# corelab-src/dacapo

Hardware: AMD Instinct MI355X
Metric: NTT/s (NTT-equivalents over one run() of the ResNet HEVM program, nt=2^14) (higher is better)
Workload: dtype u64; 1 GPU; ResNet-20 (SiLU) HEVM program traced from the reference's examples/benchmarks/ResNet.py with its resnet20.silu.model weights, nt=2^14 slots, N=2^15, 14 x 60-bit primes (SEAL_HEVM.cpp:39-53); one independent ciphertext stream per GPU; streams_per_gpu=1, parallelism=replicas x1 (no collective in the op path)

## Files before the change

### dacapo_amd/csrc/hevm_vm.hip

```cpp
#include "hevm_vm.hpp"

#include "../../include/dacapo_ckks.h"
#include "c_api_types.hpp"
#include "chacha.hpp"
#include "seal_serial.hpp"

#include <math.h>
#include <string.h>
#include <sys/random.h>

#include <algorithm>
#include <cmath>
#include <chrono>
#include <fstream>
#include <iostream>

namespace dacapo {

constexpr int kVmThreads = 256;

constexpr int kRngCoefs = 8;

__device__ __forceinline__ int rng_cbd(u64 w)
{
// ... 393 lines not shown
        abort();
    }
    const int bits = (int)option(OPT_PRIME_BITS);
    ctx.reset(new Context(logN, K, bits, primes, ksp, alpha));
    ctx->ensure_scratch();
    encoder.reset(new HostEncoder(logN));
    use_plan = option(OPT_PLAN) != 0;
    plan_graph = option(OPT_PLAN_GRAPH) != 0;
    plan_dag = option(OPT_PLAN_GRAPH) == 2;
    plan_lanes = option(OPT_PLAN_LANES) >= 2 ? 2 : 1;
    host_encoder = option(OPT_HOST_ENCODER) != 0;
    fold_rescale_into_boot = option(OPT_FOLD_RESCALE_BOOT) != 0;
    lazy_sums = option(OPT_HYB_LAZY_SUM) != 0;
    double_hoist = (lazy_sums && option(OPT_HYB_DOUBLE_HOIST) != 0) || ks_lazy == 2;
    max_batch = std::max(1, (int)option(OPT_MAX_BATCH));
    chain_fusion = option(OPT_CHAIN_FUSION) != 0;
    secret_weight = (int)option(OPT_SECRET_HW);
    boot_secret_weight = (int)option(OPT_BOOT_SECRET_HW);
    rot_compose = option(OPT_ROT_COMPOSE) != 0;
    online_encode = option(OPT_ONLINE_ENCODE) != 0 && use_plan && !host_encoder;
    lanes.resize(1);
    DC_HIP_CHECK(hipStreamCreateWithFlags(&lanes[0].stream, hipStreamNonBlocking));
    lanes[0].ws = ctx->ws0;
    lanes[0].boot_plain.d = dalloc((size_t)ctx->max_level() * ctx->N);
    lanes[0].boot_plain.level = ctx->max_level();
    DC_HIP_CHECK(vm_malloc(&d_epoch, 8));
    DC_HIP_CHECK(hipMemset(d_epoch, 0, 8));
    cur = 0;
}

// ... 1228 lines not shown
    const CrtTables &tb = crt_tables(ell);
    u64 *pt = W().ks_tmp;
    u64 *lohi = W().ks_digits;
    f_irows_decrypt(c, src, keys.sk, ell, pt, S());
    launch_ntt_cols_inv(c, pt, (long)N, ell, nullptr, 0, 0, S());
    const CrtDev cd{ tb.inv, tb.mmod, tb.hmod, tb.hdig, tb.mdbl };
    DC_LAUNCH(reencode_kernel, dim3((unsigned)((N / 2 + kVmThreads) / kVmThreads)), dim3(kVmThreads), 0, S(), lohi,
                       lohi + N, pt, ell, N, c.d_mods, cd, new_scale / src_scale);
    Plain ptx{ lanes[cur].boot_plain.d, target_level, new_scale };
    DC_LAUNCH(lift_i128_kernel, dim3((unsigned)(N / kVmThreads), (unsigned)target_level), dim3(kVmThreads), 0, S(),
                       ptx.d, lohi, lohi + N, N, c.d_mods);
    launch_ntt(c, false, ptx.d, (long)N, target_level, nullptr, 0, 0, S());
    encrypt_plain(dst, ptx);
}

void HEVM::plan_zero_encrypt(int first, int B, int t, hipStream_t s)
{
    Context &c = *ctx;
    const size_t N = c.N;
    const int cnt = t + 1;
    if (!keys.pk) {
        fprintf(stderr, "[dacapo_amd] bootstrap: this VM has no public key\n");
        abort();
    }
    Plan &P = plan;
    DC_LAUNCH(sample_enc_batch_kernel, dim3((unsigned)(N / (kRngCoefs * kVmThreads)), (unsigned)(3 * B)), dim3(kVmThreads), 0, s,
                       P.boot_ue, N, cnt, rng.secret, ((u64)1 << 32) + (u64)first, c.d_mods, d_epoch);
    launch_ntt(c, false, P.boot_ue, (long)N, 3 * cnt * B, nullptr, 0, cnt, s);
    DC_LAUNCH(pk_encrypt_batch_kernel, dim3((unsigned)(N / (2 * kVmThreads)), (unsigned)cnt, (unsigned)(2 * B)), dim3(kVmThreads),
                       0, s, P.boot_tmp, keys.pk, (long)c.K * (long)N, P.boot_ue, cnt, N, c.d_mods);
    b_rescale(c, P.ws[0], P.d_boot_rs + first, B, cnt, s);
}

void HEVM::plan_boot_step(int first, int B, int ell, int t, int lane, hipStream_t s, const Handoff &h)
{
    Context &c = *ctx;
    const size_t N = c.N;
    if (!keys.sk) {
        fprintf(stderr, "[dacapo_amd] bootstrap: needs a full VM (secret + public key)\n");
        abort();
    }
    Plan &P = plan;
    const BootItem *items = P.d_boot + first;
    const CrtTables &tb = crt_tables(ell);
    const CrtDev cd{ tb.inv, tb.mmod, tb.hmod, tb.hdig, tb.mdbl };
    u64 *pt = P.boot_pt[lane], *ptx = P.boot_ptx[lane];
// ... 26 lines not shown
    case 9: op_mulcp(op.dst, op.lhs, op.rhs); break;
    case 10: op_bootstrap(op.dst, op.lhs, op.rhs); break;
    case kOpConj: op_conj(op.dst, op.lhs); break;
    case kOpModRaise: op_modraise(op.dst, op.lhs, op.rhs); break;
    case kOpSetScale: op_setscale(op.dst, op.lhs, op.rhs); break;
    case kOpKeySwitch: op_keyswitch(op.dst, op.lhs, op.rhs); break;
    default: break;
    }
}

void HEVM::execute()
{
    memset(op_counts, 0, sizeof(op_counts));
    n_keyswitch = n_ntt = 0;
    n_hops = n_decomp = 0, n_fold = 0;
    t_bootstrap = 0.0;
    int i = (int)((header.hevm_header_size + config.config_body_length) / 8), j = 0;
    for (const WireOp &op : ops) {
        if (debug) {
            std::cout << std::endl;
            std::cout << std::oct << i++ << " " << std::dec << j++ << std::endl;
            std::cout << "opcode [" << op.opcode << "], dst [" << op.dst << "], lhs [" << op.lhs << "], rhs [" << op.rhs << "]"
                      << std::endl;
        }
        if (op.opcode <= 10) op_counts[op.opcode]++;
        if (op.opcode == 0 || (op.opcode > 10 && (op.opcode < kOpConj || op.opcode > kOpKeySwitch))) continue;
        dispatch(op);
    }
    bump_epoch(S());
}
// ... 351 lines not shown
    if (ntts) *ntts = h->n_ntt;
}

void hevm_last_run_hoist_stats(void *vm, int64_t *hops, int64_t *decompositions)
{
    auto h = V(vm);
    if (hops) *hops = h->n_hops;
    if (decompositions) *decompositions = h->n_decomp;
}

void hevm_last_run_fold_rescale_stats(void *vm, int64_t *pairs)
{
    if (pairs) *pairs = V(vm)->n_fold;
}

int64_t hevm_plan_lazy_groups(void *vm, int32_t *out, int64_t cap)
{
    auto h = V(vm);
    if (!h->plan.ready) return -1;
    std::vector<int32_t> flat;
    for (const auto &p : h->plan.pops)
        if (!p.dead && p.kind == HEVM::P_ROTSUM) {
            flat.push_back((int32_t)p.ops.size());
            flat.insert(flat.end(), p.ops.begin(), p.ops.end());
        }
    if (out && cap >= (int64_t)flat.size()) memcpy(out, flat.data(), flat.size() * sizeof(int32_t));
    return (int64_t)flat.size();
}

void hevm_destroy(void *vm)
// ... 11 lines not shown
```

### dacapo_amd/csrc/hevm_vm.hpp

```cpp
#pragma once
#include "wire_parse.hpp"
#include <complex>
#include <deque>
#include <map>
#include <set>
#include <memory>
#include <string>
#include <unordered_set>
#include <vector>

#include "../../include/hevm_abi.h"
#include "chacha.hpp"
#include "seal_serial.hpp"
#include "kernels.hpp"
#include "encoder.hpp"
#include "plan.hpp"

namespace dacapo {

struct VmAllocs {
    std::unordered_set<void *> live;
};
extern thread_local VmAllocs *g_vm_allocs;
template <class T>
// ... 125 lines not shown
        bool dead = false;
        int wave = 0, step = -1;
        int op = -1;
        bool direct = false;
        std::vector<u32> elts;
        std::vector<const u64 *> keys;
        std::vector<int> ops;
        std::vector<int> plains;
    };
    struct Step {
        PopKind kind;
        int level = 0, first = 0, count = 0;
        int target = 0;
        int wave = 0, lane = 0;
        Handoff h;
        int fused_consumer = -1;
        bool fold_rs = false;
        int gfirst = 0, gcount = 0;
        int unique = 0;
        std::vector<const u64 *> reads, writes;
    };
    struct Plan {
        bool ready = false;
        std::vector<Val> vals;
        std::vector<Pop> pops;
        std::vector<Step> steps;
        std::vector<int> final_val;
        KsItem *d_ks = nullptr;
        MulItem *d_mul = nullptr;
        MulRsItem *d_mulrs = nullptr;
// ... 6 lines not shown
        CtView *d_cont_other = nullptr;
        struct EncGroup { int wave, level, first, count; u64 *out; };
        std::vector<EncGroup> enc_groups;
        EncItem *d_enc_items = nullptr;
        u64 *enc_arena = nullptr;
        double2 *enc_scratch = nullptr;
        int *d_enc_overflow = nullptr;
        size_t enc_arena_bytes = 0, enc_scratch_bytes = 0;
        std::vector<EwItem> h_ew;
        std::vector<u64 *> handoff_bufs;
        size_t n_fused = 0;
        BootItem *d_boot = nullptr;
        RsItem *d_boot_rs = nullptr;
        size_t zenc_bytes = 0;
        u64 *zenc = nullptr, *boot_ue = nullptr, *boot_tmp = nullptr, *boot_pt[2] = { nullptr, nullptr }, *boot_ptx[2] = { nullptr, nullptr };
        struct BootChunk { int first, count, target; };
        std::vector<BootChunk> boot_chunks;
        BatchWs ws[2];
        std::vector<hipEvent_t> events;
        std::vector<u64 *> pool;
        int64_t n_keyswitch = 0, n_ntt = 0;
        int64_t n_hops = 0, n_decomp = 0;
        int64_t n_fold = 0;
        size_t launches = 0, max_live = 0;
        hipGraph_t graph = nullptr;
        hipGraphExec_t graph_exec = nullptr;
    } plan;
    bool plan_graph = true;
    bool plan_dag = false;
    void capture_plan();
    bool capture_plan_dag();
    void issue_step(const Step &st, hipStream_t q);
    void drop_plan_graph();
    void issue_plan(hipStream_t s);
    bool use_plan = true;
    bool test_zero_enc = false;
    int max_batch = 64;
    std::vector<u64 *> home;
    int streams = 1, sel = 0;
    std::vector<u64 *> reg_base;
    void set_streams(int n);
    void select_stream(int s);
    void build_plan();
    void run_plan();
    void boot_item(CtView src, int src_level, double src_scale, hevm_ctxt &dst, int target_level);
    void plan_zero_encrypt(int first, int B, int t, hipStream_t s);
    void plan_boot_step(int first, int B, int ell, int t, int lane, hipStream_t s, const Handoff &h);
    bool rot_compose = false;
    std::vector<int> compose_rotation(int steps) const;
    mutable std::vector<int> rot_offsets;
    mutable std::set<int> rot_offset_set;
    mutable size_t rot_offsets_epoch = (size_t)-1;
    int boot_secret_weight = 0;
    int secret_weight = 0;
    bool ks_hoist = false;
    int ks_lazy = 0;
    bool ks_fold_rescale = false;
    KsItem *d_hoist_items = nullptr;
    void rotate_hop_vm(CtView dst, CtView src, u32 elt, const u64 *key, int ell);
    bool chain_fusion = true;
    hipStream_t aux_stream = nullptr;
    bool double_hoist = false;
    double *dh_consts = nullptr;
    std::map<int, EncItem> dh_items;
    void ensure_special_limbs(const std::vector<int> &plain_regs);
    bool lazy_sums = false;
    bool fold_rescale_into_boot = false;
    int plan_lanes = 2;
    void bump_epoch(hipStream_t s);

    int64_t op_counts[11] = { 0 };
    int64_t n_keyswitch = 0, n_ntt = 0;
    int64_t n_hops = 0, n_decomp = 0;
    int64_t n_fold = 0;
    double t_bootstrap = 0.0;

    VmAllocs allocs;
    HEVM() { g_vm_allocs = &allocs; }
    void destroy_device_state();
    size_t key_elems() const { return (size_t)ctx->key_digits() * 2 * ctx->K * ctx->N; }
    void init_context(int logN, int K, const u64 *primes, int dir_ksp = 0, int dir_alpha = 0);
    void generate_keys(const RngKeys &rng, bool secret, bool pub, bool eval);
    void gen_kswitch_key(u64 *key, const u64 *new_key, u64 key_id);
    void gen_kswitch_key_in(Context &c, u64 *key, const u64 *key_sk, const u64 *new_key, u64 key_id);
    void fill_sparse_secret(u64 *dst, int weight, u32 domain);
    void generate_boot_switch_keys();
    size_t swk_down_elems() const { return (size_t)2 * (1 + ctx->ksp) * ctx->N; }
    void add_galois_key(u32 elt);
    void save_keys(const std::string &dir);
// ... 37 lines not shown
```

### dacapo_amd/csrc/options.cpp

```cpp
#include "options.hpp"

#include "../../include/hevm_abi.h"

#include <stdio.h>
#include <stdlib.h>
#include <string.h>

namespace dacapo {

struct OptDef {
    const char *name;
    long long def;
};
static const OptDef kDefs[OPT_COUNT] = {
    { "logn", 15 },
    { "primes", 14 },
    { "prime_bits", 60 },
    { "ks_special", 1 },
    { "ks_alpha", 0 },
    { "secret_hw", 0 },
    { "boot_secret_hw", 0 },
    { "rot_compose", 0 },
    { "plan", 1 },
    { "plan_graph", 1 },
    { "plan_lanes", 2 },
    { "plan_aux_min_cost", 3 },
    { "max_batch", 64 },
    { "chain_fusion", 1 },
    { "host_encoder", 0 },
    { "online_encode", 0 },
    { "fold_rescale_boot", 0 },
    { "hyb_mfma", 1 },
    { "hyb_fuse", 2 },
    { "hyb_lazy_sum", 0 },
    { "hyb_double_hoist", 0 },
    { "ks_hoist", 0 },
    { "ks_lazy_sum", 0 },
    { "ks_fold_rescale", 0 },
    { "seal_compr", 0 },
    { "trace", 0 },
    { "step_profile", 0 },
    { "small_tile_wgs", -1 },
// ... 129 lines not shown
```

### dacapo_amd/csrc/options.hpp

```cpp
#pragma once

namespace dacapo {

enum Opt : int {
    OPT_LOGN,
    OPT_PRIMES,
    OPT_PRIME_BITS,
    OPT_KS_SPECIAL,
    OPT_KS_ALPHA,
    OPT_SECRET_HW,
    OPT_BOOT_SECRET_HW,
    OPT_ROT_COMPOSE,
    OPT_PLAN,
    OPT_PLAN_GRAPH,
    OPT_PLAN_LANES,
    OPT_PLAN_AUX_MIN_COST,
    OPT_MAX_BATCH,
    OPT_CHAIN_FUSION,
    OPT_HOST_ENCODER,
    OPT_ONLINE_ENCODE,
    OPT_FOLD_RESCALE_BOOT,
    OPT_HYB_MFMA,
    OPT_HYB_FUSE,
    OPT_HYB_LAZY_SUM,
    OPT_HYB_DOUBLE_HOIST,
    OPT_KS_HOIST,
    OPT_KS_LAZY_SUM,
    OPT_KS_FOLD_RESCALE,
    OPT_SEAL_COMPR,
    OPT_TRACE,
    OPT_STEP_PROFILE,
    OPT_SMALL_TILE_WGS,
// ... 25 lines not shown
```

### dacapo_amd/csrc/plan_exec.hip

```cpp
#include <math.h>
#include <string.h>

#include <algorithm>
#include <chrono>
#include <map>
#include <functional>
#include <queue>
#include <set>
#include <tuple>

#include "hevm_vm.hpp"

namespace dacapo {

#define ks_ntts(ell) ks_ntt_count(c, (ell))

template <class T>
static T *upload(const std::vector<T> &v)
{
    T *d = nullptr;
    DC_HIP_CHECK(vm_malloc(&d, std::max<size_t>(v.size(), 1) * sizeof(T)));
    if (!v.empty()) DC_HIP_CHECK(hipMemcpy(d, v.data(), v.size() * sizeof(T), hipMemcpyHostToDevice));
    return d;
}

void HEVM::build_plan()
{
    Context &c = *ctx;
    const size_t N = c.N;
    Plan &P = plan;
    for (u64 *b : P.handoff_bufs) (void)vm_free(b);
    P.handoff_bufs.clear();
    for (void *p : { (void *)P.d_enc_items, (void *)P.enc_arena, (void *)P.enc_scratch, (void *)P.d_enc_overflow })
        if (p) (void)vm_free(p);
    P.d_enc_items = nullptr, P.enc_arena = nullptr, P.enc_scratch = nullptr, P.d_enc_overflow = nullptr;
    P.enc_groups.clear(), P.enc_arena_bytes = P.enc_scratch_bytes = 0;
    if (P.d_cont_other) (void)vm_free(P.d_cont_other), P.d_cont_other = nullptr;
    if (P.d_mulrs) (void)vm_free(P.d_mulrs), P.d_mulrs = nullptr;
    for (void *p : { (void *)P.d_ks, (void *)P.d_mul, (void *)P.d_rs, (void *)P.d_ew, (void *)P.d_sum, (void *)P.d_sum_srcs, (void *)P.d_sumg, (void *)P.d_sumg_srcs, (void *)P.d_boot,
                     (void *)P.d_boot_rs, (void *)P.zenc, (void *)P.boot_ue, (void *)P.boot_tmp, (void *)P.boot_pt[0], (void *)P.boot_ptx[0],
                     (void *)P.boot_pt[1], (void *)P.boot_ptx[1] })
        if (p) (void)vm_free(p);
    P.d_boot = nullptr, P.d_boot_rs = nullptr, P.zenc = P.boot_ue = P.boot_tmp = nullptr;
    P.boot_pt[0] = P.boot_pt[1] = P.boot_ptx[0] = P.boot_ptx[1] = nullptr;
    P.boot_chunks.clear();
    if (P.graph_exec) (void)hipGraphExecDestroy(P.graph_exec);
    if (P.graph) (void)hipGraphDestroy(P.graph);
    P.graph_exec = nullptr, P.graph = nullptr;
    P.vals.clear(), P.pops.clear(), P.steps.clear();
    P.n_keyswitch = P.n_ntt = 0;
    P.n_hops = P.n_decomp = 0, P.n_fold = 0;
    const size_t nreg = ciphers.size();
    const int S = streams;
    std::vector<int> cur(nreg, -1);
    auto new_val = [&](int level, double scale) {
        Val v;
        v.level = level, v.scale = scale, v.root = (int)P.vals.size();
        P.vals.push_back(v);
        return (int)P.vals.size() - 1;
    };
// ... 529 lines not shown
            if (!ok) continue;
            bp = order;
            if (B.fold_rs) {
                std::vector<int> &rs = fold_pops.at(bi);
                for (size_t k = 0; k < bp.size(); k++) rs[k] = fold_rs_of.at(bp[k]);
            }
            Step &A = P.steps[(size_t)ai];
            A.fused_consumer = (int)bi;
            A.h.cont = B.kind == P_RESCALE ? CONT_RS : B.kind == P_BOOT ? CONT_BOOT : CONT_MUL;
            if (B.kind == P_MULCC)
                for (size_t k = 0; k < bp.size(); k++) mul_fused_src[(size_t)bp[k]] = which2[k];
            P.n_fused++;
        }
    }
    if (plan_lanes >= 2) {
        auto cost = [](const Step &st) { return st.kind == P_ROT || st.kind == P_MULCC || st.kind == P_ROTSUM ? 8 : st.kind == P_BOOT ? 5 : st.kind == P_RESCALE ? 3 : 1; };
        for (size_t a = 0; a < P.steps.size();) {
            size_t b = a;
            while (b < P.steps.size() && P.steps[b].wave == P.steps[a].wave) b++;
            std::vector<size_t> idx;
            for (size_t i = a; i < b; i++) idx.push_back(i);
            std::stable_sort(idx.begin(), idx.end(), [&](size_t x, size_t y) { return cost(P.steps[x]) > cost(P.steps[y]); });
            int load[2] = { 0, 0 };
            for (size_t i : idx) {
                const int lane = load[1] < load[0] ? 1 : 0;
                P.steps[i].lane = lane, load[lane] += cost(P.steps[i]);
            }
            if (load[1] < (int)option(OPT_PLAN_AUX_MIN_COST))
                for (size_t i = a; i < b; i++) P.steps[i].lane = 0;
            a = b;
        }
// ... 363 lines not shown
        for (int pi : step_pops[s]) {
            const Pop &p = O[(size_t)pi];
            for (int v : p.srcs) st.reads.push_back(V[(size_t)V[(size_t)v].root].buf);
            st.writes.push_back(V[(size_t)V[(size_t)p.dst].root].buf);
        }
        if (st.fold_rs)
            for (int pi : fold_pops.at(s)) st.writes.push_back(V[(size_t)V[(size_t)O[(size_t)pi].dst].root].buf);
        if (st.fused_consumer >= 0 && st.h.cont == CONT_MUL)
            for (int pi : step_pops[(size_t)st.fused_consumer])
                for (int v : O[(size_t)pi].srcs) st.reads.push_back(V[(size_t)V[(size_t)v].root].buf);
        for (auto *vec : { &st.reads, &st.writes }) {
            std::sort(vec->begin(), vec->end());
            vec->erase(std::unique(vec->begin(), vec->end()), vec->end());
        }
    }
    if (!h_boot_pops.empty()) {
        const size_t nb = h_boot_pops.size(), slot = (size_t)2 * boot_tmax * N;
        DC_HIP_CHECK(vm_malloc(&P.zenc, nb * slot * sizeof(u64)));
        P.zenc_bytes = nb * slot * sizeof(u64);
        std::vector<int> order(nb);
        for (size_t i = 0; i < nb; i++) order[i] = (int)i;
        std::stable_sort(order.begin(), order.end(), [&](int a, int b) {
            return O[(size_t)h_boot_pops[(size_t)a].first].target_level < O[(size_t)h_boot_pops[(size_t)b].first].target_level;
        });
        const size_t bc = std::min<size_t>(nb, (size_t)std::max(max_batch, 1));
        const size_t cmax = (size_t)boot_tmax + 1;
        DC_HIP_CHECK(vm_malloc(&P.boot_ue, bc * 3 * cmax * N * sizeof(u64)));
        DC_HIP_CHECK(vm_malloc(&P.boot_tmp, bc * 2 * cmax * N * sizeof(u64)));
        for (int ln = 0; ln < plan_lanes; ln++) {
            DC_HIP_CHECK(vm_malloc(&P.boot_pt[ln], std::max<size_t>(need_bpt, 1) * N * sizeof(u64)));
            DC_HIP_CHECK(vm_malloc(&P.boot_ptx[ln], std::max<size_t>(need_bptx, 1) * N * sizeof(u64)));
        }
        std::vector<BootItem> h_boot(nb);
        std::vector<RsItem> h_brs(nb);
        for (size_t k = 0; k < nb;) {
            const int t = O[(size_t)h_boot_pops[(size_t)order[k]].first].target_level;
            size_t e = k;
            while (e < nb && e - k < bc && O[(size_t)h_boot_pops[(size_t)order[e]].first].target_level == t) e++;
            P.boot_chunks.push_back({ (int)k, (int)(e - k), t });
            for (size_t j = k; j < e; j++) {
                const size_t item = (size_t)order[j];
                u64 *z = P.zenc + item * slot;
                h_brs[j] = RsItem{ CtView{ P.boot_tmp + (j - k) * 2 * (size_t)(t + 1) * N, (long)(t + 1) * (long)N }, CtView{ z, (long)t * (long)N } };
            }
            need_d = std::max(need_d, (e - k) * 2), need_m = std::max(need_m, (e - k) * 2 * (size_t)(t + 1));
            P.launches += 7;
            k = e;
        }
        for (size_t item = 0; item < nb; item++) {
            const Pop &p = O[(size_t)h_boot_pops[item].first];
            const int q = h_boot_pops[item].second;
            const double new_scale = V[(size_t)p.dst].scale;
            BootItem bi{ view(p.srcs[0], q), view(p.dst, q), P.zenc + item * slot, 1.0 };
            double src_scale;
            if (p.boot_drop >= 0) {
                src_scale = p.boot_src_scale * (double)c.primes[(size_t)p.boot_drop];
            } else
                src_scale = V[(size_t)p.srcs[0]].scale;
            bi.ratio = new_scale / src_scale;
            if (p.rs_sum) {
                bi.first = (int)h_srcs.size(), bi.count = (int)p.srcs.size();
                for (size_t k = 0; k < p.srcs.size(); k++) {
// ... 32 lines not shown
                        const Pop &mp = O[(size_t)pi];
                        const int w = mul_fused_src[(size_t)pi], other = mp.srcs[(size_t)(1 - w)];
                        h_cont_other.push_back(other == mp.srcs[(size_t)w] ? CtView{ nullptr, 0 } : view(other, q));
                    }
            }
        }
        P.d_cont_other = upload(h_cont_other);
        for (size_t ai = 0; ai < P.steps.size(); ai++)
            if (P.steps[ai].fused_consumer >= 0 && P.steps[ai].h.cont == CONT_MUL) P.steps[ai].h.other = P.d_cont_other + other_first[ai];
    }
    auto alloc = [&](size_t limbs) {
        u64 *d = nullptr;
        DC_HIP_CHECK(vm_malloc(&d, std::max<size_t>(limbs, 1) * N * sizeof(u64)));
        return d;
    };
    for (int ln = 0; ln < 2; ln++) {
        BatchWs &w = P.ws[ln];
        for (void *p : { (void *)w.target, (void *)w.digits, (void *)w.ext, (void *)w.acc, (void *)w.tmp })
            if (p) (void)vm_free(p);
        w = BatchWs{};
        if (ln >= plan_lanes) continue;
        w.target = alloc(need_t), w.digits = alloc(need_d), w.ext = alloc(need_e);
        w.acc = alloc(need_a), w.tmp = alloc(need_m);
    }
    {
        size_t aux_waves = 0;
        for (size_t i = 0; i < P.steps.size(); i++)
            if (P.steps[i].lane == 1 && (i == 0 || P.steps[i - 1].wave != P.steps[i].wave || P.steps[i - 1].lane != 1)) aux_waves++;
        while (P.events.size() < 2 * aux_waves + 2) {
            hipEvent_t e;
            DC_HIP_CHECK(hipEventCreateWithFlags(&e, hipEventDisableTiming));
            P.events.push_back(e);
        }
        if (aux_waves && !aux_stream) DC_HIP_CHECK(hipStreamCreateWithFlags(&aux_stream, hipStreamNonBlocking));
    }
    P.n_keyswitch *= S, P.n_ntt *= S;
    P.ready = true;
    if (plan_graph) capture_plan();
    if (option(OPT_TRACE)) {
        static const char *kn[] = { "rot", "mulcc", "rescale", "sum", "neg", "mulp", "addp", "copy", "boot", "modraise", "rotsum" };
        size_t nsteps[kPopKinds] = { 0 }, nitems[kPopKinds] = { 0 };
        std::map<std::pair<int, int>, std::pair<size_t, size_t>> ks;
        for (const Step &st : P.steps) {
            nsteps[st.kind]++, nitems[st.kind] += (size_t)st.count;
            if (st.kind == P_ROT || st.kind == P_MULCC || st.kind == P_RESCALE || st.kind == P_BOOT || st.kind == P_ROTSUM) {
                auto &e = ks[{ (int)st.kind, st.level }];
                e.first++, e.second += (size_t)st.count;
            }
        }
// ... 79 lines not shown
    case P_NEG: b_ew(c, EwOp::Neg, P.d_ew + st.first, st.count, 2, 2, st.level, q); break;
    case P_COPY: b_ew(c, EwOp::Copy, P.d_ew + st.first, st.count, 2, 2, st.level, q); break;
    case P_MODRAISE: modraise(c, w.digits, P.h_ew.data() + st.first, st.count, st.target, q, P.d_ew + st.first); break;
    case P_MULP: b_ew(c, EwOp::Mul, P.d_ew + st.first, st.count, 2, 1, st.level, q); break;
    case P_ADDP: b_add_plain(c, P.d_ew + st.first, st.count, st.level, q); break;
    case P_BOOT: plan_boot_step(st.first, st.count, st.level, st.target, st.lane, q, st.h); break;
    }
}

void HEVM::issue_plan(hipStream_t s)
{
    Context &c = *ctx;
    Plan &P = plan;
    if (test_zero_enc) {
        if (P.zenc) DC_HIP_CHECK(hipMemsetAsync(P.zenc, 0, P.zenc_bytes, s));
    } else
        for (const Plan::BootChunk &bc : P.boot_chunks) plan_zero_encrypt(bc.first, bc.count, bc.target, s);
    const bool step_profile = option(OPT_STEP_PROFILE) != 0 && !plan_graph;
    std::map<std::tuple<int, int, int>, std::pair<int, double>> prof;
    double wave_max = 0, wave_sum = 0, crit_path = 0, all_steps = 0;
    size_t waves_seen = 0, wide_waves = 0;
    size_t ev = 0, eg = 0;
    for (size_t a = 0; a < P.steps.size();) {
        size_t b = a;
        bool has_aux = false;
        while (b < P.steps.size() && P.steps[b].wave == P.steps[a].wave) has_aux |= P.steps[b].lane == 1, b++;
        for (; eg < P.enc_groups.size() && P.enc_groups[eg].wave <= P.steps[a].wave; eg++) {
            const Plan::EncGroup &g = P.enc_groups[eg];
            enc_batch(c, enc_tables, online.d_consts, P.d_enc_items + g.first, g.count, g.level, P.enc_scratch, g.out, P.d_enc_overflow, s);
        }
        if (has_aux) {
            DC_HIP_CHECK(hipEventRecord(P.events[ev], s));
            DC_HIP_CHECK(hipStreamWaitEvent(aux_stream, P.events[ev], 0));
            ev++;
        }
        for (size_t i = a; i < b; i++) {
            const Step &st = P.steps[i];
            hipStream_t q = st.lane ? aux_stream : s;
            issue_step(st, q);
            if (step_profile) {
                static auto t_prev = std::chrono::steady_clock::now();
                if (i == 0) {
                    DC_HIP_CHECK(hipStreamSynchronize(s));
                    t_prev = std::chrono::steady_clock::now();
                }
                DC_HIP_CHECK(hipStreamSynchronize(q));
                const auto t1 = std::chrono::steady_clock::now();
                const int bucket = st.count <= 1 ? 1 : st.count <= 2 ? 2 : st.count <= 4 ? 4 : st.count <= 8 ? 8 : st.count <= 32 ? 32 : 128;
                auto &e = prof[std::make_tuple((int)st.kind, st.level, bucket)];
                const double dt = std::chrono::duration<double>(t1 - t_prev).count();
                e.first++, e.second += dt;
                wave_max = std::max(wave_max, dt), wave_sum += dt;
                t_prev = t1;
            }
        }
        if (has_aux) {
            DC_HIP_CHECK(hipEventRecord(P.events[ev], aux_stream));
            DC_HIP_CHECK(hipStreamWaitEvent(s, P.events[ev], 0));
            ev++;
        }
        if (step_profile) {
            crit_path += wave_max, all_steps += wave_sum, waves_seen++, wide_waves += (b - a) > 1;
            wave_max = wave_sum = 0;
        }
        a = b;
    }
    bump_epoch(s);
    if (step_profile) {
        static const char *kn[] = { "rot", "mulcc", "rescale", "sum", "neg", "mulp", "addp", "copy", "boot", "modraise", "rotsum" };
        double total = 0;
        for (auto &kv : prof) total += kv.second.second;
        fprintf(stderr, "[dacapo_amd] step profile (synchronised after every step): %.2f ms in %zu steps\n", total * 1e3, P.steps.size());
        fprintf(stderr, "[dacapo_amd]   %zu waves, %zu of them with more than one step; sum of all steps %.2f ms, sum over waves of the longest step %.2f ms "
                        "(= %.1f %% of the serial time)\n", waves_seen, wide_waves, all_steps * 1e3, crit_path * 1e3, 100.0 * crit_path / all_steps);
        for (auto &kv : prof)
            fprintf(stderr, "[dacapo_amd]   %-8s level %2d  batch<=%-3d  %5d steps  %8.3f ms  %7.2f us/step\n", kn[std::get<0>(kv.first)],
                    std::get<1>(kv.first), std::get<2>(kv.first), kv.second.first, kv.second.second * 1e3,
                    kv.second.second * 1e6 / kv.second.first);
    }
}
// ... 57 lines not shown
                DC_HIP_CHECK(hipGraphKernelNodeGetParams(cur, &kp));
                DC_HIP_CHECK(hipGraphAddKernelNode(&nw, main, dp, nd, &kp));
            } else if (ty == hipGraphNodeTypeMemset) {
                hipMemsetParams mp;
                DC_HIP_CHECK(hipGraphMemsetNodeGetParams(cur, &mp));
                DC_HIP_CHECK(hipGraphAddMemsetNode(&nw, main, dp, nd, &mp));
            } else
                ok = false;
            tail = nw;
            auto it = next.find(cur);
            cur = it == next.end() ? nullptr : it->second;
        }
        (void)hipGraphDestroy(g);
        return tail;
    };
    hipGraphNode_t zenc_tail = add_unit([&](hipStream_t s) {
        if (test_zero_enc) {
            if (P.zenc) DC_HIP_CHECK(hipMemsetAsync(P.zenc, 0, P.zenc_bytes, s));
        } else
            for (const Plan::BootChunk &bc : P.boot_chunks) plan_zero_encrypt(bc.first, bc.count, bc.target, s);
    }, {});
    struct Ref { int lane = -1; long seq = -1; hipGraphNode_t node = nullptr; };
    std::map<const u64 *, Ref> writer;
    std::map<const u64 *, Ref> reader[2];
    Ref lane_tail[2] = { Ref{ 0, 0, zenc_tail }, Ref{ 1, 0, zenc_tail } };
    long seq = 0;
    for (size_t i = 0; i < P.steps.size() && ok; i++) {
        const Step &st = P.steps[i];
        const int other = 1 - st.lane;
        Ref cross;
        auto need = [&](const Ref &r) {
            if (r.node && r.lane == other && r.seq > cross.seq) cross = r;
        };
        for (const u64 *b : st.reads) {
            auto it = writer.find(b);
            if (it != writer.end()) need(it->second);
        }
        for (const u64 *b : st.writes) {
            auto it = writer.find(b);
            if (it != writer.end()) need(it->second);
            auto rt = reader[other].find(b);
            if (rt != reader[other].end()) need(rt->second);
        }
        std::vector<hipGraphNode_t> deps{ lane_tail[st.lane].node };
        if (cross.node) deps.push_back(cross.node);
        const hipGraphNode_t tail = add_unit([&](hipStream_t s) { issue_step(st, s); }, deps);
        if (!tail) continue;
        const Ref me{ st.lane, ++seq, tail };
        lane_tail[st.lane] = me;
        for (const u64 *b : st.reads) reader[st.lane][b] = me;
        for (const u64 *b : st.writes) writer[b] = me;
    }
    if (ok) (void)add_unit([&](hipStream_t s) { bump_epoch(s); }, { lane_tail[0].node, lane_tail[1].node });
    if (!ok) {
        (void)hipGraphDestroy(main);
        return false;
    }
    P.graph = main;
    DC_HIP_CHECK(hipGraphInstantiate(&P.graph_exec, P.graph, nullptr, nullptr, 0));
    return true;
}

void HEVM::drop_plan_graph()
{
    Plan &P = plan;
    if (P.graph_exec) (void)hipGraphExecDestroy(P.graph_exec);
    if (P.graph) (void)hipGraphDestroy(P.graph);
    P.graph_exec = nullptr, P.graph = nullptr;
}

void HEVM::run_plan()
{
    if (!plan.ready) build_plan();
    Context &c = *ctx;
    Plan &P = plan;
    cur = 0;
    hipStream_t s = S();
    memset(op_counts, 0, sizeof(op_counts));
    for (const WireOp &op : ops)
        if (op.opcode <= 10) op_counts[op.opcode]++;
    n_keyswitch = P.n_keyswitch, n_ntt = P.n_ntt;
    n_hops = P.n_hops, n_decomp = P.n_decomp, n_fold = P.n_fold;
    t_bootstrap = 0.0;
    const long ps = (long)c.K * (long)c.N;
    if (plan_graph) {
        capture_plan();
        if (P.graph_exec)
            DC_HIP_CHECK(hipGraphLaunch(P.graph_exec, s));
        else
            issue_plan(s);
    } else
        issue_plan(s);
    DC_HIP_CHECK(hipStreamSynchronize(s));
    if (P.d_enc_overflow) {
        int overflow = 0;
        DC_HIP_CHECK(hipMemcpy(&overflow, P.d_enc_overflow, sizeof(int), hipMemcpyDeviceToHost));
        if (overflow) {
// ... 17 lines not shown
```

### dacapo_amd/runner.py

```python
from __future__ import annotations

import contextlib
import ctypes
import re
import weakref
from pathlib import Path

import numpy as np

from . import LIB_PATH

lw = None


def reinit_lw():
    global lw
    if lw is None:
        lw = bind_vm_lib(LIB_PATH)
    return lw


_vm_libs: dict = {}


# ... 52 lines not shown
    L.hevm_keys_replaced.argtypes = [ctypes.c_void_p]
    L.hevm_boot_switch_keys.argtypes = [ctypes.c_void_p, ctypes.POINTER(ctypes.c_void_p), ctypes.POINTER(ctypes.c_void_p),
                                        ctypes.POINTER(ctypes.c_int)]
    L.hevm_boot_switch_keys.restype = ctypes.c_int
    L.hevm_galois_key.argtypes = [ctypes.c_void_p, ctypes.c_uint32]
    L.hevm_galois_key.restype = ctypes.c_void_p
    L.hevm_plain.argtypes = [ctypes.c_void_p, ctypes.c_int64, ctypes.POINTER(ctypes.c_int32), ctypes.POINTER(ctypes.c_double)]
    L.hevm_plain.restype = ctypes.c_void_p
    L.hevm_plain_special.argtypes = [ctypes.c_void_p, ctypes.c_int64]
    L.hevm_plain_special.restype = ctypes.c_void_p
    L.hevm_load_mem.argtypes = [ctypes.c_void_p, ctypes.c_char_p, ctypes.c_uint64, ctypes.c_char_p, ctypes.c_uint64]
    L.hevm_last_run_stats.argtypes = [ctypes.c_void_p, ctypes.POINTER(ctypes.c_int64), ctypes.POINTER(ctypes.c_int64),
                                       ctypes.POINTER(ctypes.c_int64)]
    L.hevm_last_run_hoist_stats.argtypes = [ctypes.c_void_p, ctypes.POINTER(ctypes.c_int64), ctypes.POINTER(ctypes.c_int64)]
    L.hevm_last_run_fold_rescale_stats.argtypes = [ctypes.c_void_p, ctypes.POINTER(ctypes.c_int64)]
    L.hevm_plan_lazy_groups.argtypes = [ctypes.c_void_p, ctypes.POINTER(ctypes.c_int32), ctypes.c_int64]
    L.hevm_plan_lazy_groups.restype = ctypes.c_int64
    L.hevm_set_streams.argtypes = [ctypes.c_void_p, ctypes.c_int]
    L.hevm_select_stream.argtypes = [ctypes.c_void_p, ctypes.c_int]
    L.hevm_last_run_bootstrap_seconds.argtypes = [ctypes.c_void_p]
    L.hevm_last_run_bootstrap_seconds.restype = ctypes.c_double
    L.hevm_plaintext_bytes.argtypes = [ctypes.c_void_p]
    L.hevm_plaintext_bytes.restype = ctypes.c_uint64
    L.hevm_destroy.argtypes = [ctypes.c_void_p]
    L.hevm_destroy.restype = None
    L.hevm_add_rotation_keys.argtypes = [ctypes.c_void_p, ctypes.POINTER(ctypes.c_int64), ctypes.c_int]
    L.hevm_save_ctxt.argtypes = [ctypes.c_void_p, ctypes.c_int64, ctypes.c_char_p]
    L.hevm_load_ctxt.argtypes = [ctypes.c_void_p, ctypes.c_int64, ctypes.c_char_p]
    bind_options(L)
    for name, value in _cli_options.items():
# ... 243 lines not shown
        while i < n:
            out.append(list(buf[i + 1 : i + 1 + buf[i]]))
            i += 1 + buf[i]
        return out

    def hoist_stats(self):
        hops, dec = ctypes.c_int64(), ctypes.c_int64()
        self.lw.hevm_last_run_hoist_stats(self.vm, ctypes.byref(hops), ctypes.byref(dec))
        return {"hops": hops.value, "decompositions": dec.value}

    def fold_rescale_stats(self):
        pairs = ctypes.c_int64()
        self.lw.hevm_last_run_fold_rescale_stats(self.vm, ctypes.byref(pairs))
        return pairs.value

    def stats(self):
        counts = (ctypes.c_int64 * 11)()
        ks, ntt = ctypes.c_int64(), ctypes.c_int64()
        self.lw.hevm_last_run_stats(self.vm, counts, ctypes.byref(ks), ctypes.byref(ntt))
        return {"op_counts": list(counts), "keyswitches": ks.value, "ntts": ntt.value,
                "bootstrap_s": float(self.lw.hevm_last_run_bootstrap_seconds(self.vm))}

    def printer(self, latency, rms, mem_usage=0.0):
        bench = re.search(r"optimized/(.*)/(.*)\.(.*)\._", self.hevm_path)
        print("======================================")
        print("---------------Option-----------------")
        if bench:
            print("compiler:", bench.group(1))
            print("benchname:", bench.group(2))
            print("waterline:", bench.group(3))
# ... 8 lines not shown
```

### include/hevm_abi.h

```cpp
#ifndef HEVM_ABI_H
#define HEVM_ABI_H

#include <stdbool.h>
#include <stdint.h>

#ifdef __cplusplus
extern "C" {
#endif
#if defined(__GNUC__)
#pragma GCC visibility push(default)
#endif

void *initFullVM(char *dir, bool device);
void *initClientVM(char *dir);
void *initServerVM(char *dir);
void create_context(char *dir);
void load(void *vm, char *constant, char *vmfile);
void loadClient(void *vm, void *is);
void encrypt(void *vm, int64_t i, double *dat, int len);
void decrypt(void *vm, int64_t i, double *dat);
void decrypt_result(void *vm, int64_t i, double *dat);
int64_t getResIdx(void *vm, int64_t i);
void *getCtxt(void *vm, int64_t id);
void preprocess(void *vm);
// ... 22 lines not shown
#endif
void *hevm_context(void *vm);
const uint64_t *hevm_relin_key(void *vm);
const uint64_t *hevm_galois_key(void *vm, uint32_t elt);
const uint64_t *hevm_public_key(void *vm);
int hevm_boot_switch_keys(void *vm, const uint64_t **down, const uint64_t **up, int *down_limbs);
int hevm_key_buffers(void *vm, uint64_t **ptrs, uint64_t *words, int cap);
uint64_t hevm_key_digest(void *vm);
void hevm_keys_replaced(void *vm);
const uint64_t *hevm_plain(void *vm, int64_t i, int32_t *level, double *scale);
const uint64_t *hevm_plain_special(void *vm, int64_t i);
void hevm_load_mem(void *vm, const void *cst, uint64_t cst_len, const void *hevm, uint64_t hevm_len);
void hevm_last_run_stats(void *vm, int64_t *op_counts , int64_t *keyswitches, int64_t *ntts);
void hevm_last_run_hoist_stats(void *vm, int64_t *hops, int64_t *decompositions);
void hevm_last_run_fold_rescale_stats(void *vm, int64_t *pairs);
int64_t hevm_plan_lazy_groups(void *vm, int32_t *out, int64_t cap);
void hevm_set_streams(void *vm, int n);
void hevm_select_stream(void *vm, int s);
double hevm_last_run_bootstrap_seconds(void *vm);
uint64_t hevm_plaintext_bytes(void *vm);
void hevm_destroy(void *vm);
void hevm_add_rotation_keys(void *vm, const int64_t *offsets, int count);
void hevm_save_ctxt(void *vm, int64_t reg, const char *path);
void hevm_load_ctxt(void *vm, int64_t reg, const char *path);

int hevm_set_option(const char *name, long long value);
long long hevm_get_option(const char *name);
void hevm_reset_options(void);

void hevm_seal_parms_id(uint64_t poly_modulus_degree, const uint64_t *primes, int count, uint64_t out[4]);
// ... 18 lines not shown
```

Baseline: 1.308 million NTT/s.

## Overlap bootstrap zero-encryptions with main-stream work on the auxiliary stream

Instead of generating every fresh zero-encryption used by bootstrapping up front on the main stream, the plan now splits them into smaller chunks, orders them by the wave that first reads them, and issues them on the auxiliary stream inside idle windows estimated from per-step costs. Bootstrap steps wait on the event of their chunk, and the graph path adds matching dependencies. A dedicated workspace is allocated for these rescales so they do not race with lane workspaces. The aim is to hide the encryption prologue behind the compute-heavy waves, at the cost of more events and cross-stream waits, smaller batches, and contention with aux-lane work.

New measurement: 1.307 million NTT/s. About the same (-0.1%).

```diff
diff --git a/dacapo_amd/csrc/hevm_vm.hip b/dacapo_amd/csrc/hevm_vm.hip
--- a/dacapo_amd/csrc/hevm_vm.hip
+++ b/dacapo_amd/csrc/hevm_vm.hip
@@ -431,6 +431,10 @@
     lazy_sums = option(OPT_HYB_LAZY_SUM) != 0;
     double_hoist = (lazy_sums && option(OPT_HYB_DOUBLE_HOIST) != 0) || ks_lazy == 2;
     max_batch = std::max(1, (int)option(OPT_MAX_BATCH));
+    zenc_overlap = option(OPT_PLAN_ZENC_OVERLAP) != 0 && plan_lanes >= 2;
+    zenc_chunk = std::max(1, (int)option(OPT_PLAN_ZENC_CHUNK));
+    zenc_head = std::max(0, (int)option(OPT_PLAN_ZENC_HEAD));
+    zenc_cost = std::max(0, (int)option(OPT_PLAN_ZENC_COST));
     chain_fusion = option(OPT_CHAIN_FUSION) != 0;
     secret_weight = (int)option(OPT_SECRET_HW);
     boot_secret_weight = (int)option(OPT_BOOT_SECRET_HW);
@@ -1689,7 +1693,7 @@
     encrypt_plain(dst, ptx);
 }
 
-void HEVM::plan_zero_encrypt(int first, int B, int t, hipStream_t s)
+void HEVM::plan_zero_encrypt(int first, int B, int t, const BatchWs &w, hipStream_t s)
 {
     Context &c = *ctx;
     const size_t N = c.N;
@@ -1704,7 +1708,7 @@
     launch_ntt(c, false, P.boot_ue, (long)N, 3 * cnt * B, nullptr, 0, cnt, s);
     DC_LAUNCH(pk_encrypt_batch_kernel, dim3((unsigned)(N / (2 * kVmThreads)), (unsigned)cnt, (unsigned)(2 * B)), dim3(kVmThreads),
                        0, s, P.boot_tmp, keys.pk, (long)c.K * (long)N, P.boot_ue, cnt, N, c.d_mods);
-    b_rescale(c, P.ws[0], P.d_boot_rs + first, B, cnt, s);
+    b_rescale(c, w, P.d_boot_rs + first, B, cnt, s);
 }
 
 void HEVM::plan_boot_step(int first, int B, int ell, int t, int lane, hipStream_t s, const Handoff &h)
@@ -1761,6 +1765,7 @@
     memset(op_counts, 0, sizeof(op_counts));
     n_keyswitch = n_ntt = 0;
     n_hops = n_decomp = 0, n_fold = 0;
+    memset(n_zenc, 0, sizeof(n_zenc));
     t_bootstrap = 0.0;
     int i = (int)((header.hevm_header_size + config.config_body_length) / 8), j = 0;
     for (const WireOp &op : ops) {
@@ -2142,6 +2147,11 @@
     if (pairs) *pairs = V(vm)->n_fold;
 }
 
+void hevm_last_run_zenc_stats(void *vm, int64_t *out)
+{
+    if (out) memcpy(out, V(vm)->n_zenc, sizeof(V(vm)->n_zenc));
+}
+
 int64_t hevm_plan_lazy_groups(void *vm, int32_t *out, int64_t cap)
 {
     auto h = V(vm);
diff --git a/dacapo_amd/csrc/hevm_vm.hpp b/dacapo_amd/csrc/hevm_vm.hpp
--- a/dacapo_amd/csrc/hevm_vm.hpp
+++ b/dacapo_amd/csrc/hevm_vm.hpp
@@ -163,6 +163,7 @@
         int target = 0;
         int wave = 0, lane = 0;
         Handoff h;
+        int zenc_chunk = -1;
         int fused_consumer = -1;
         bool fold_rs = false;
         int gfirst = 0, gcount = 0;
@@ -199,9 +200,12 @@
         RsItem *d_boot_rs = nullptr;
         size_t zenc_bytes = 0;
         u64 *zenc = nullptr, *boot_ue = nullptr, *boot_tmp = nullptr, *boot_pt[2] = { nullptr, nullptr }, *boot_ptx[2] = { nullptr, nullptr };
-        struct BootChunk { int first, count, target; };
+        struct BootChunk { int first, count, target; int before = 0; bool window = false, head = false; };
         std::vector<BootChunk> boot_chunks;
+        bool zenc_overlap = false;
+        int64_t n_zenc[4] = { 0, 0, 0, 0 };
         BatchWs ws[2];
+        BatchWs zws;
         std::vector<hipEvent_t> events;
         std::vector<u64 *> pool;
         int64_t n_keyswitch = 0, n_ntt = 0;
@@ -220,6 +224,10 @@
     void issue_plan(hipStream_t s);
     bool use_plan = true;
     bool test_zero_enc = false;
+    bool zenc_overlap = false;
+    int zenc_chunk = 8;
+    int zenc_head = 0;
+    int zenc_cost = 100;
     int max_batch = 64;
     std::vector<u64 *> home;
     int streams = 1, sel = 0;
@@ -229,7 +237,7 @@
     void build_plan();
     void run_plan();
     void boot_item(CtView src, int src_level, double src_scale, hevm_ctxt &dst, int target_level);
-    void plan_zero_encrypt(int first, int B, int t, hipStream_t s);
+    void plan_zero_encrypt(int first, int B, int t, const BatchWs &w, hipStream_t s);
     void plan_boot_step(int first, int B, int ell, int t, int lane, hipStream_t s, const Handoff &h);
     bool rot_compose = false;
     std::vector<int> compose_rotation(int steps) const;
@@ -258,6 +266,7 @@
     int64_t n_keyswitch = 0, n_ntt = 0;
     int64_t n_hops = 0, n_decomp = 0;
     int64_t n_fold = 0;
+    int64_t n_zenc[4] = { 0, 0, 0, 0 };
     double t_bootstrap = 0.0;
 
     VmAllocs allocs;
diff --git a/dacapo_amd/csrc/options.cpp b/dacapo_amd/csrc/options.cpp
--- a/dacapo_amd/csrc/options.cpp
+++ b/dacapo_amd/csrc/options.cpp
@@ -26,6 +26,10 @@
     { "plan_lanes", 2 },
     { "plan_aux_min_cost", 3 },
     { "max_batch", 64 },
+    { "plan_zenc_overlap", 1 },
+    { "plan_zenc_chunk", 8 },
+    { "plan_zenc_head", 0 },
+    { "plan_zenc_cost", 100 },
     { "chain_fusion", 1 },
     { "host_encoder", 0 },
     { "online_encode", 0 },
diff --git a/dacapo_amd/csrc/options.hpp b/dacapo_amd/csrc/options.hpp
--- a/dacapo_amd/csrc/options.hpp
+++ b/dacapo_amd/csrc/options.hpp
@@ -16,6 +16,10 @@
     OPT_PLAN_LANES,
     OPT_PLAN_AUX_MIN_COST,
     OPT_MAX_BATCH,
+    OPT_PLAN_ZENC_OVERLAP,
+    OPT_PLAN_ZENC_CHUNK,
+    OPT_PLAN_ZENC_HEAD,
+    OPT_PLAN_ZENC_COST,
     OPT_CHAIN_FUSION,
     OPT_HOST_ENCODER,
     OPT_ONLINE_ENCODE,
diff --git a/dacapo_amd/csrc/plan_exec.hip b/dacapo_amd/csrc/plan_exec.hip
--- a/dacapo_amd/csrc/plan_exec.hip
+++ b/dacapo_amd/csrc/plan_exec.hip
@@ -22,6 +22,11 @@
     DC_HIP_CHECK(vm_malloc(&d, std::max<size_t>(v.size(), 1) * sizeof(T)));
     if (!v.empty()) DC_HIP_CHECK(hipMemcpy(d, v.data(), v.size() * sizeof(T), hipMemcpyHostToDevice));
     return d;
+}
+
+static int step_cost(HEVM::PopKind k)
+{
+    return k == HEVM::P_ROT || k == HEVM::P_MULCC || k == HEVM::P_ROTSUM ? 8 : k == HEVM::P_BOOT ? 5 : k == HEVM::P_RESCALE ? 3 : 1;
 }
 
 void HEVM::build_plan()
@@ -44,6 +49,8 @@
     P.d_boot = nullptr, P.d_boot_rs = nullptr, P.zenc = P.boot_ue = P.boot_tmp = nullptr;
     P.boot_pt[0] = P.boot_pt[1] = P.boot_ptx[0] = P.boot_ptx[1] = nullptr;
     P.boot_chunks.clear();
+    P.zenc_overlap = false;
+    memset(P.n_zenc, 0, sizeof(P.n_zenc));
     if (P.graph_exec) (void)hipGraphExecDestroy(P.graph_exec);
     if (P.graph) (void)hipGraphDestroy(P.graph);
     P.graph_exec = nullptr, P.graph = nullptr;
@@ -603,7 +610,7 @@
         }
     }
     if (plan_lanes >= 2) {
-        auto cost = [](const Step &st) { return st.kind == P_ROT || st.kind == P_MULCC || st.kind == P_ROTSUM ? 8 : st.kind == P_BOOT ? 5 : st.kind == P_RESCALE ? 3 : 1; };
+        auto cost = [](const Step &st) { return step_cost(st.kind); };
         for (size_t a = 0; a < P.steps.size();) {
             size_t b = a;
             while (b < P.steps.size() && P.steps[b].wave == P.steps[a].wave) b++;
@@ -997,6 +1004,7 @@
             vec->erase(std::unique(vec->begin(), vec->end()), vec->end());
         }
     }
+    size_t zneed_d = 0, zneed_m = 0;
     if (!h_boot_pops.empty()) {
         const size_t nb = h_boot_pops.size(), slot = (size_t)2 * boot_tmax * N;
         DC_HIP_CHECK(vm_malloc(&P.zenc, nb * slot * sizeof(u64)));
@@ -1006,7 +1014,10 @@
         std::stable_sort(order.begin(), order.end(), [&](int a, int b) {
             return O[(size_t)h_boot_pops[(size_t)a].first].target_level < O[(size_t)h_boot_pops[(size_t)b].first].target_level;
         });
-        const size_t bc = std::min<size_t>(nb, (size_t)std::max(max_batch, 1));
+        P.zenc_overlap = zenc_overlap;
+        const size_t head_items = P.zenc_overlap ? std::min<size_t>(nb, (size_t)zenc_head) : 0;
+        const size_t bc_over = std::min<size_t>(nb, (size_t)std::max(P.zenc_overlap ? std::min(max_batch, zenc_chunk) : max_batch, 1));
+        const size_t bc = head_items ? std::min<size_t>(nb, (size_t)std::max(max_batch, 1)) : bc_over;
         const size_t cmax = (size_t)boot_tmax + 1;
         DC_HIP_CHECK(vm_malloc(&P.boot_ue, bc * 3 * cmax * N * sizeof(u64)));
         DC_HIP_CHECK(vm_malloc(&P.boot_tmp, bc * 2 * cmax * N * sizeof(u64)));
@@ -1019,16 +1030,91 @@
         for (size_t k = 0; k < nb;) {
             const int t = O[(size_t)h_boot_pops[(size_t)order[k]].first].target_level;
             size_t e = k;
-            while (e < nb && e - k < bc && O[(size_t)h_boot_pops[(size_t)order[e]].first].target_level == t) e++;
-            P.boot_chunks.push_back({ (int)k, (int)(e - k), t });
+            const bool at_head = k < head_items;
+            while (e < nb && e - k < (at_head ? bc : bc_over) && (!at_head || e < head_items) && O[(size_t)h_boot_pops[(size_t)order[e]].first].target_level == t) e++;
+            P.boot_chunks.push_back(Plan::BootChunk{ (int)k, (int)(e - k), t });
+            P.boot_chunks.back().head = at_head;
             for (size_t j = k; j < e; j++) {
                 const size_t item = (size_t)order[j];
                 u64 *z = P.zenc + item * slot;
                 h_brs[j] = RsItem{ CtView{ P.boot_tmp + (j - k) * 2 * (size_t)(t + 1) * N, (long)(t + 1) * (long)N }, CtView{ z, (long)t * (long)N } };
             }
-            need_d = std::max(need_d, (e - k) * 2), need_m = std::max(need_m, (e - k) * 2 * (size_t)(t + 1));
+            zneed_d = std::max(zneed_d, (e - k) * 2), zneed_m = std::max(zneed_m, (e - k) * 2 * (size_t)(t + 1));
             P.launches += 7;
             k = e;
+        }
+        {
+            std::vector<int> chunk_of(nb, 0), first_group(P.boot_chunks.size(), -1);
+            for (size_t ci = 0; ci < P.boot_chunks.size(); ci++)
+                for (int j = 0; j < P.boot_chunks[ci].count; j++) chunk_of[(size_t)order[(size_t)(P.boot_chunks[ci].first + j)]] = (int)ci;
+            struct Group { size_t a, b; bool aux; int main_cost; };
+            std::vector<Group> groups;
+            for (size_t a = 0; a < P.steps.size();) {
+                Group g{ a, a, false, 0 };
+                while (g.b < P.steps.size() && P.steps[g.b].wave == P.steps[a].wave) {
+                    const Step &st = P.steps[g.b++];
+                    g.aux |= st.lane == 1;
+                    if (st.lane == 0) g.main_cost += step_cost(st.kind);
+                    if (st.kind == P_BOOT)
+                        for (int k = 0; k < st.count; k++) {
+                            int &fg = first_group[(size_t)chunk_of[(size_t)(st.first + k)]];
+                            if (fg < 0) fg = (int)groups.size();
+                        }
+                }
+                groups.push_back(g);
+                a = g.b;
+            }
+            std::vector<int> new_pos(P.boot_chunks.size());
+            {
+                std::vector<int> by(P.boot_chunks.size());
+                for (size_t i = 0; i < by.size(); i++) by[i] = (int)i;
+                auto rank = [&](int x) { return P.boot_chunks[(size_t)x].head ? -1 : first_group[(size_t)x]; };
+                if (P.zenc_overlap) std::stable_sort(by.begin(), by.end(), [&](int x, int y) { return rank(x) < rank(y); });
+                std::vector<Plan::BootChunk> sorted;
+                std::vector<int> fg;
+                for (size_t i = 0; i < by.size(); i++) new_pos[(size_t)by[i]] = (int)i, sorted.push_back(P.boot_chunks[(size_t)by[i]]), fg.push_back(first_group[(size_t)by[i]]);
+                P.boot_chunks = sorted, first_group = fg;
+            }
+            for (Step &st : P.steps)
+                if (st.kind == P_BOOT)
+                    for (int k = 0; k < st.count; k++) st.zenc_chunk = std::max(st.zenc_chunk, new_pos[(size_t)chunk_of[(size_t)(st.first + k)]]);
+            P.n_zenc[0] = (int64_t)P.boot_chunks.size();
+            if (P.zenc_overlap) {
+                const long long pct = zenc_cost;
+                auto chunk_cost = [&](const Plan::BootChunk &ch) { return (long long)(7 + ch.count * (ch.target + 1) / 4) * pct / 100; };
+                size_t next = 0;
+                while (next < P.boot_chunks.size() && P.boot_chunks[next].head) next++;
+                long long owed = 0;
+                for (size_t g = 0; g < groups.size() && next < P.boot_chunks.size(); g++) {
+                    for (; next < P.boot_chunks.size() && first_group[next] <= (int)g; next++)
+                        P.boot_chunks[next].before = (int)g, owed += chunk_cost(P.boot_chunks[next]);
+                    if (groups[g].aux) {
+                        owed = 0;
+                        continue;
+                    }
+                    long long window = 0;
+                    for (size_t h = g; h < groups.size() && !groups[h].aux; h++) window += groups[h].main_cost;
+                    for (; next < P.boot_chunks.size() && owed + chunk_cost(P.boot_chunks[next]) <= window; next++)
+                        P.boot_chunks[next].before = (int)g, P.boot_chunks[next].window = true, owed += chunk_cost(P.boot_chunks[next]);
+                    owed = std::max<long long>(owed - groups[g].main_cost, 0);
+                }
+                for (size_t ci = 0; ci < P.boot_chunks.size(); ci++) P.n_zenc[1] += !P.boot_chunks[ci].head && first_group[ci] > 0;
+                for (const Step &st : P.steps)
+                    if (st.kind == P_BOOT && st.lane == 0 && !P.boot_chunks[(size_t)st.zenc_chunk].head) P.n_zenc[2]++, P.n_zenc[3]++;
+                if (option(OPT_TRACE)) {
+                    size_t in_window = 0, at_head = 0;
+                    for (const Plan::BootChunk &ch : P.boot_chunks) in_window += ch.window, at_head += ch.head;
+                    fprintf(stderr, "[dacapo_amd] plan: zero-encryptions: %zu chunks at the head (%zu items), %zu chunks of at most %zu items on the auxiliary "
+                                    "stream, %zu in idle windows, %zu at their deadline, %lld away from the head; %lld opcode-10 steps wait across streams\n",
+                            at_head, head_items, P.boot_chunks.size() - at_head, bc_over, in_window, P.boot_chunks.size() - at_head - in_window,
+                            (long long)P.n_zenc[1], (long long)P.n_zenc[3]);
+                    if (option(OPT_TRACE) >= 2)
+                        for (size_t ci = 0; ci < P.boot_chunks.size(); ci++)
+                            fprintf(stderr, "[dacapo_amd] plan:   chunk %zu: %d items to %d primes ahead of wave %d (%s), first read in wave %d\n", ci,
+                                    P.boot_chunks[ci].count, P.boot_chunks[ci].target, P.steps[groups[(size_t)P.boot_chunks[ci].before].a].wave,
+                                    P.boot_chunks[ci].head ? "head" : P.boot_chunks[ci].window ? "window" : "deadline", P.steps[groups[(size_t)first_group[ci]].a].wave);
+                }
+            }
         }
         for (size_t item = 0; item < nb; item++) {
             const Pop &p = O[(size_t)h_boot_pops[item].first];
@@ -1091,11 +1177,15 @@
         DC_HIP_CHECK(vm_malloc(&d, std::max<size_t>(limbs, 1) * N * sizeof(u64)));
         return d;
     };
-    for (int ln = 0; ln < 2; ln++) {
-        BatchWs &w = P.ws[ln];
+    for (int ln = 0; ln < 3; ln++) {
+        BatchWs &w = ln < 2 ? P.ws[ln] : P.zws;
         for (void *p : { (void *)w.target, (void *)w.digits, (void *)w.ext, (void *)w.acc, (void *)w.tmp })
             if (p) (void)vm_free(p);
         w = BatchWs{};
+        if (ln == 2) {
+            if (zneed_d) w.digits = alloc(zneed_d), w.tmp = alloc(zneed_m);
+            continue;
+        }
         if (ln >= plan_lanes) continue;
         w.target = alloc(need_t), w.digits = alloc(need_d), w.ext = alloc(need_e);
         w.acc = alloc(need_a), w.tmp = alloc(need_m);
@@ -1104,12 +1194,13 @@
         size_t aux_waves = 0;
         for (size_t i = 0; i < P.steps.size(); i++)
             if (P.steps[i].lane == 1 && (i == 0 || P.steps[i - 1].wave != P.steps[i].wave || P.steps[i - 1].lane != 1)) aux_waves++;
-        while (P.events.size() < 2 * aux_waves + 2) {
+        const size_t zenc_events = P.zenc_overlap ? P.boot_chunks.size() + 2 : 0;
+        while (P.events.size() < 2 * aux_waves + 2 + zenc_events) {
             hipEvent_t e;
             DC_HIP_CHECK(hipEventCreateWithFlags(&e, hipEventDisableTiming));
             P.events.push_back(e);
         }
-        if (aux_waves && !aux_stream) DC_HIP_CHECK(hipStreamCreateWithFlags(&aux_stream, hipStreamNonBlocking));
+        if ((aux_waves || zenc_events) && !aux_stream) DC_HIP_CHECK(hipStreamCreateWithFlags(&aux_stream, hipStreamNonBlocking));
     }
     P.n_keyswitch *= S, P.n_ntt *= S;
     P.ready = true;
@@ -1219,8 +1310,17 @@
     Plan &P = plan;
     if (test_zero_enc) {
         if (P.zenc) DC_HIP_CHECK(hipMemsetAsync(P.zenc, 0, P.zenc_bytes, s));
-    } else
-        for (const Plan::BootChunk &bc : P.boot_chunks) plan_zero_encrypt(bc.first, bc.count, bc.target, s);
+    } else if (!P.zenc_overlap)
+        for (const Plan::BootChunk &bc : P.boot_chunks) plan_zero_encrypt(bc.first, bc.count, bc.target, P.zws, s);
+    const bool overlap = P.zenc_overlap && !test_zero_enc && !P.boot_chunks.empty();
+    const size_t zev0 = P.events.size() - (P.boot_chunks.size() + 2);
+    size_t next_chunk = 0, group = 0;
+    for (; overlap && next_chunk < P.boot_chunks.size() && P.boot_chunks[next_chunk].head; next_chunk++)
+        plan_zero_encrypt(P.boot_chunks[next_chunk].first, P.boot_chunks[next_chunk].count, P.boot_chunks[next_chunk].target, P.zws, s);
+    if (overlap) {
+        DC_HIP_CHECK(hipEventRecord(P.events[zev0], s));
+        DC_HIP_CHECK(hipStreamWaitEvent(aux_stream, P.events[zev0], 0));
+    }
     const bool step_profile = option(OPT_STEP_PROFILE) != 0 && !plan_graph;
     std::map<std::tuple<int, int, int>, std::pair<int, double>> prof;
     double wave_max = 0, wave_sum = 0, crit_path = 0, all_steps = 0;
@@ -1234,6 +1334,12 @@
             const Plan::EncGroup &g = P.enc_groups[eg];
             enc_batch(c, enc_tables, online.d_consts, P.d_enc_items + g.first, g.count, g.level, P.enc_scratch, g.out, P.d_enc_overflow, s);
         }
+        for (; overlap && next_chunk < P.boot_chunks.size() && P.boot_chunks[next_chunk].before <= (int)group; next_chunk++) {
+            const Plan::BootChunk &bc = P.boot_chunks[next_chunk];
+            plan_zero_encrypt(bc.first, bc.count, bc.target, P.zws, aux_stream);
+            DC_HIP_CHECK(hipEventRecord(P.events[zev0 + 1 + next_chunk], aux_stream));
+        }
+        group++;
         if (has_aux) {
             DC_HIP_CHECK(hipEventRecord(P.events[ev], s));
             DC_HIP_CHECK(hipStreamWaitEvent(aux_stream, P.events[ev], 0));
@@ -1242,6 +1348,8 @@
         for (size_t i = a; i < b; i++) {
             const Step &st = P.steps[i];
             hipStream_t q = st.lane ? aux_stream : s;
+            if (overlap && st.kind == P_BOOT && st.lane == 0 && !P.boot_chunks[(size_t)st.zenc_chunk].head)
+                DC_HIP_CHECK(hipStreamWaitEvent(s, P.events[zev0 + 1 + (size_t)st.zenc_chunk], 0));
             issue_step(st, q);
             if (step_profile) {
                 static auto t_prev = std::chrono::steady_clock::now();
@@ -1269,6 +1377,11 @@
             wave_max = wave_sum = 0;
         }
         a = b;
+    }
+    if (overlap) {
+        const size_t e = zev0 + 1 + P.boot_chunks.size();
+        DC_HIP_CHECK(hipEventRecord(P.events[e], aux_stream));
+        DC_HIP_CHECK(hipStreamWaitEvent(s, P.events[e], 0));
     }
     bump_epoch(s);
     if (step_profile) {
@@ -1356,12 +1469,20 @@
         (void)hipGraphDestroy(g);
         return tail;
     };
-    hipGraphNode_t zenc_tail = add_unit([&](hipStream_t s) {
-        if (test_zero_enc) {
-            if (P.zenc) DC_HIP_CHECK(hipMemsetAsync(P.zenc, 0, P.zenc_bytes, s));
-        } else
-            for (const Plan::BootChunk &bc : P.boot_chunks) plan_zero_encrypt(bc.first, bc.count, bc.target, s);
-    }, {});
+    const bool overlap = P.zenc_overlap && !test_zero_enc && !P.boot_chunks.empty();
+    std::vector<hipGraphNode_t> chunk_tail;
+    hipGraphNode_t zenc_tail = nullptr;
+    if (overlap)
+        for (const Plan::BootChunk &bc : P.boot_chunks)
+            chunk_tail.push_back(add_unit([&](hipStream_t s) { plan_zero_encrypt(bc.first, bc.count, bc.target, P.zws, s); },
+                                          { chunk_tail.empty() ? nullptr : chunk_tail.back() }));
+    else
+        zenc_tail = add_unit([&](hipStream_t s) {
+            if (test_zero_enc) {
+                if (P.zenc) DC_HIP_CHECK(hipMemsetAsync(P.zenc, 0, P.zenc_bytes, s));
+            } else
+                for (const Plan::BootChunk &bc : P.boot_chunks) plan_zero_encrypt(bc.first, bc.count, bc.target, P.zws, s);
+        }, {});
     struct Ref { int lane = -1; long seq = -1; hipGraphNode_t node = nullptr; };
     std::map<const u64 *, Ref> writer;
     std::map<const u64 *, Ref> reader[2];
@@ -1386,6 +1507,7 @@
         }
         std::vector<hipGraphNode_t> deps{ lane_tail[st.lane].node };
         if (cross.node) deps.push_back(cross.node);
+        if (overlap && st.kind == P_BOOT) deps.push_back(chunk_tail.at((size_t)st.zenc_chunk));
         const hipGraphNode_t tail = add_unit([&](hipStream_t s) { issue_step(st, s); }, deps);
         if (!tail) continue;
         const Ref me{ st.lane, ++seq, tail };
@@ -1393,7 +1515,7 @@
         for (const u64 *b : st.reads) reader[st.lane][b] = me;
         for (const u64 *b : st.writes) writer[b] = me;
     }
-    if (ok) (void)add_unit([&](hipStream_t s) { bump_epoch(s); }, { lane_tail[0].node, lane_tail[1].node });
+    if (ok) (void)add_unit([&](hipStream_t s) { bump_epoch(s); }, { lane_tail[0].node, lane_tail[1].node, chunk_tail.empty() ? nullptr : chunk_tail.back() });
     if (!ok) {
         (void)hipGraphDestroy(main);
         return false;
@@ -1423,6 +1545,7 @@
         if (op.opcode <= 10) op_counts[op.opcode]++;
     n_keyswitch = P.n_keyswitch, n_ntt = P.n_ntt;
     n_hops = P.n_hops, n_decomp = P.n_decomp, n_fold = P.n_fold;
+    memcpy(n_zenc, P.n_zenc, sizeof(n_zenc));
     t_bootstrap = 0.0;
     const long ps = (long)c.K * (long)c.N;
     if (plan_graph) {
diff --git a/dacapo_amd/runner.py b/dacapo_amd/runner.py
--- a/dacapo_amd/runner.py
+++ b/dacapo_amd/runner.py
@@ -90,6 +90,7 @@
                                        ctypes.POINTER(ctypes.c_int64)]
     L.hevm_last_run_hoist_stats.argtypes = [ctypes.c_void_p, ctypes.POINTER(ctypes.c_int64), ctypes.POINTER(ctypes.c_int64)]
     L.hevm_last_run_fold_rescale_stats.argtypes = [ctypes.c_void_p, ctypes.POINTER(ctypes.c_int64)]
+    L.hevm_last_run_zenc_stats.argtypes = [ctypes.c_void_p, ctypes.POINTER(ctypes.c_int64)]
     L.hevm_plan_lazy_groups.argtypes = [ctypes.c_void_p, ctypes.POINTER(ctypes.c_int32), ctypes.c_int64]
     L.hevm_plan_lazy_groups.restype = ctypes.c_int64
     L.hevm_set_streams.argtypes = [ctypes.c_void_p, ctypes.c_int]
@@ -363,6 +364,11 @@
         self.lw.hevm_last_run_fold_rescale_stats(self.vm, ctypes.byref(pairs))
         return pairs.value
 
+    def zenc_stats(self):
+        out = (ctypes.c_int64 * 4)()
+        self.lw.hevm_last_run_zenc_stats(self.vm, out)
+        return {"chunks": out[0], "away_from_head": out[1], "cross_stream_steps": out[2], "waits": out[3]}
+
     def stats(self):
         counts = (ctypes.c_int64 * 11)()
         ks, ntt = ctypes.c_int64(), ctypes.c_int64()
diff --git a/include/hevm_abi.h b/include/hevm_abi.h
--- a/include/hevm_abi.h
+++ b/include/hevm_abi.h
@@ -60,6 +60,7 @@
 void hevm_last_run_stats(void *vm, int64_t *op_counts , int64_t *keyswitches, int64_t *ntts);
 void hevm_last_run_hoist_stats(void *vm, int64_t *hops, int64_t *decompositions);
 void hevm_last_run_fold_rescale_stats(void *vm, int64_t *pairs);
+void hevm_last_run_zenc_stats(void *vm, int64_t *out );
 int64_t hevm_plan_lazy_groups(void *vm, int32_t *out, int64_t cap);
 void hevm_set_streams(void *vm, int n);
 void hevm_select_stream(void *vm, int s);
```
